# haoxiangsnr/Wave-U-Net-for-Speech-Enhancement

Measured on AMD Instinct MI355X. Metric: 16384-sample frames/sec fwd+bwd, 12-level Wave-U-Net, higher is better.
Workload: dtype f32 (levels >= 16 samples: 3 x f16 MFMA on hi/lo fp16 halves, fp32 accumulate; the rest f32 MFMA); 1 GPU; unet_basic 12-level, 16384-sample frames, batch=64 per GPU, fp32, training-mode forward + smooth_l1 + backward + fused HIP Adam step (BASELINE.json configs[2]; configs[3] when n_gpus>1); global_batch=64, frame=16384, parallelism=dp1

## Files before the change

### wave-u-net-for-speech-enhancement_amd/csrc/wunet_backward.cpp

```cpp
#include "wunet_host.h"
#include "wunet_elementwise.h"
#include "wunet_tiny.h"
#include "wunet_h3_elem.h"
#include "wunet_input_grad.h"

using namespace wunet_host;

namespace {
#ifndef WUNET_EMU
__global__ void stamp_kernel(unsigned long long* p) { *p = wall_clock64(); }
unsigned long long* g_stamps = nullptr;
bool stamps_on()
{
    static const bool on = getenv("WUNET_STAMP") != nullptr;
    if (on && !g_stamps && (hipMalloc(&g_stamps, 128 * sizeof(unsigned long long)) != hipSuccess || hipMemset(g_stamps, 0, 128 * sizeof(unsigned long long)) != hipSuccess)) g_stamps = nullptr;
    return on && g_stamps;
}
#define WUNET_STAMP(stream_, slot_) { if (stamps_on()) hipLaunchKernelGGL(stamp_kernel, dim3(1), dim3(1), 0, stream_, g_stamps + (slot_)); }
#else
#define WUNET_STAMP(stream_, slot_) {}
#endif

bool dx_stays_split(const wunet_ctx* c, int i)
{
    if (i < 1 || i > c->n) return false;
    const LayerPlan& l = c->ly[i];
    return l.d.ksplit > 1 && l.L >= 4 && c->ly[i - 1].L >= 4;
}

bool enc_gz_off()
{
    static const bool off = getenv("WUNET_NO_ENC_GZ") != nullptr;
    return off;
}
bool pa_swap_on()
{
    static const int on = getenv("WUNET_PA_SWAP") ? atoi(getenv("WUNET_PA_SWAP")) : 1;
    return on != 0;
}

bool bwd_tiny(const wunet_ctx* c, int i) { return c->ly[i].L < 4; }
bool bwd_one_block(const wunet_ctx* c, int i) { return c->ly[i].a_split == 1 && (size_t)c->B * c->ly[i].L <= 4 * WUNET_THREADS; }
bool bwd_fuse(const wunet_ctx* c, int i) { return !bwd_tiny(c, i) && i < c->NL - 1 && !(i > 0 && c->ly[i].h3d) && bwd_one_block(c, i); }

bool upt_handoff(const wunet_ctx* c, int q) { return q > c->n && q < c->NL && c->ly[q].upt; }
bool upt_handoff_sound(const wunet_ctx* c, int q)
{
    const LayerPlan& l = c->ly[q];
    return l.src0 == q - 1 && l.h3d && l.d.ksplit == 1 && c->ly[q - 1].h3d && !bwd_tiny(c, q - 1) && !bwd_fuse(c, q - 1);
}

enum { DG_NONE = 0, DG_H3 = 1, DG_SCALAR = 2, DG_FP32 = 3 };
struct BwdLayerPlan {
    bool tiny;
    bool fuse;
    bool gz_h3;
    bool gz_in_wgrad;
    bool e0;
    int pa_mode;
    const char* pa_name;
    double g_src_bytes;
    bool stores_g;
    bool swap;
    bool g1_split;
    bool fin_in_gz;
    int gz_mode;
    int dgrad;
    bool dx_split, dx_sum;
    bool upt;
    double pa_bytes() const { return 4.0 + g_src_bytes + (stores_g ? 4.0 : 0.0); }
    double gz_bytes() const { return 4.0 + (gz_mode == GZ_G ? 4.0 : g_src_bytes); }
};
BwdLayerPlan bwd_layer_plan(const wunet_ctx* c, int i)
{
    const LayerPlan& l = c->ly[i];
    const int NL = c->NL, n = c->n;
    BwdLayerPlan q{};
    q.tiny = bwd_tiny(c, i);
    q.fuse = bwd_fuse(c, i);
    q.gz_h3 = i > 0 && l.h3d;
    q.gz_in_wgrad = i == 0 && !q.tiny && !l.h3d && !l.h3w && l.w.wsplit && !bwd_one_block(c, i);
    q.e0 = c->e0 && q.gz_in_wgrad && !q.fuse && l.cin == 1 && l.taps == 15 && l.L >= 16 && !dx_stays_split(c, 1) && n >= 1;
    const bool recompute = q.gz_h3 && !q.fuse && !q.tiny;
    q.stores_g = true;
    if (i == NL - 1) {
        q.pa_mode = A_HEAD; q.pa_name = "pass_a_kernel<HEAD>"; q.g_src_bytes = 0.0; q.gz_mode = GZ_HEAD;
        q.stores_g = !recompute;
    } else if (i >= n && upt_handoff(c, i + 1)) {
        q.pa_mode = A_UPH; q.pa_name = "pass_a_kernel<UPH>"; q.g_src_bytes = 4.0; q.gz_mode = GZ_UPH;
        q.stores_g = false;
    } else if (i >= n) {
        q.pa_mode = A_UP; q.pa_name = "pass_a_kernel<UP>"; q.g_src_bytes = 8.0; q.gz_mode = GZ_G;
    } else {
        q.g1_split = dx_stays_split(c, i + 1);
        q.pa_mode = A_ENC; q.pa_name = q.e0 ? "pass_a_kernel<ENC, e0>" : "pass_a_kernel<ENC>"; q.g_src_bytes = 6.0; q.gz_mode = GZ_ENC;
        q.stores_g = !(!enc_gz_off() && recompute && !q.g1_split) && !q.e0;
    }
    if (q.stores_g) q.gz_mode = GZ_G;
    q.swap = pa_swap_on() && l.a_split > 1 && !q.tiny;
    q.fin_in_gz = !q.fuse && q.gz_h3 && l.a_split * l.cout <= WUNET_GZ_FIN_LOADS && l.cout <= WUNET_GZ_FIN_C;
    q.dgrad = i == 0 ? DG_NONE : l.h3d ? DG_H3 : q.tiny ? DG_SCALAR : DG_FP32;
    q.dx_split = q.dgrad != DG_NONE && q.dgrad != DG_SCALAR && l.d.ksplit > 1;
    q.dx_sum = q.dx_split && !dx_stays_split(c, i);
    q.upt = upt_handoff(c, i);
    return q;
}

int first_layer_gz_source(const wunet_ctx* c)
{
    const BwdLayerPlan q = bwd_layer_plan(c, 0);
    return q.e0 ? IG_ENC : q.gz_in_wgrad ? IG_G : IG_GZ;
}

struct BwdCall {
    wunet_ctx* c; float* ws; const float* const* params; float* const* grads; const float* noisy;
    hipStream_t st, sd;
    wunet_ctx::Side* side;
};

int head_backward(const BwdCall& k, void* workspace, const float* enhanced, const float* grad_enhanced)
{
    wunet_ctx* c = k.c; float* ws = k.ws; const hipStream_t st = k.st;
    if (k.side->packed_ws == workspace && k.sd != st) {
        k.side->packed_ws = nullptr;
        if (hipStreamWaitEvent(st, k.side->ev_pack, 0) != hipSuccess) return fail(WUNET_E_RUNTIME, "waiting for the weight packs failed");
    } else {
        k.side->packed_ws = nullptr;
        const int rc = launch_backward_packs(c, k.params, ws, st);
        if (rc) return rc;
    }
    const LayerPlan& l = c->ly[c->NL - 1];
    HeadBwdArgs h{};
    h.z = ws + l.z; h.a = ws + l.a; h.s = ws + l.s; h.in = k.noisy; h.out = enhanced; h.gout = grad_enhanced;
    h.gh = ws + c->gh_off; h.part = ws + c->hpart_off; h.B = c->B; h.C = c->ci; h.T = c->T; h.logT = ilog2(c->T);
    WUNET_LAUNCH(head_bwd_kernel, dim3(c->head_blocks), dim3(WUNET_THREADS), 0, st, h);
    WUNET_CHECK_LAUNCH();
    return WUNET_OK;
}

int pass_a(const BwdCall& k, int i, const BwdLayerPlan& q, int fz)
{
    wunet_ctx* c = k.c; float* ws = k.ws; const hipStream_t st = k.st;
    const int NL = c->NL, n = c->n;
    const LayerPlan& l = c->ly[i];
    PassAArgs p{};
    p.z = ws + l.z; p.a = ws + l.a; p.s = ws + l.s; p.mean = ws + l.mean; p.rstd = ws + l.rstd;
    p.gpre = q.stores_g ? ws + l.g : nullptr; p.part = ws + c->bpart_off; p.pmax = q.gz_h3 ? ws + c->bmax_off : nullptr;
    p.B = c->B; p.C = l.cout; p.L = l.L; p.logL = l.logL; p.Lt = l.Lt;
    p.swap = q.swap ? 1 : 0;
    const dim3 ga(p.swap ? l.a_split : l.cout, p.swap ? l.cout : l.a_split);
    if (q.fuse) {
        p.gamma = k.params[4 * i + 2]; p.dgamma = k.grads[4 * i + 2]; p.dbeta = k.grads[4 * i + 3]; p.dbias = k.grads[4 * i + 1];
        p.k1 = ws + l.k1; p.k2 = ws + l.k2; p.k3 = ws + l.k3; p.count = (double)c->B * l.Lt; p.frozen = fz;
    }
    prof_begin(st, q.pa_name, 0.0, (double)c->B * l.cout * l.L * q.pa_bytes() + (q.pa_mode == A_HEAD ? 4.0 * c->B * l.L : 0.0));
    if (q.pa_mode == A_HEAD) {
        p.g0 = ws + c->gh_off; p.g1 = k.params[4 * NL]; p.hpart = ws + c->hpart2_off;
        WUNET_LAUNCH(pass_a_kernel<A_HEAD>, ga, dim3(WUNET_THREADS), 0, st, p);
    } else if (q.pa_mode == A_UPH) {
        const LayerPlan& nx = c->ly[i + 1];
        p.g0 = ws + nx.dxh; p.sp = ws + nx.usp; p.ntiles = (int)(((size_t)c->B * nx.L + 255) / 256); p.tpr = l.L >> 7;
        WUNET_LAUNCH(pass_a_kernel<A_UPH>, ga, dim3(WUNET_THREADS), 0, st, p);
    } else if (q.pa_mode == A_UP) {
        const LayerPlan& nx = c->ly[i + 1];
        p.g0 = ws + nx.dx; p.Cg0 = nx.cin;
        p.up_scale = (float)(l.Lt - 1) / (float)(2 * l.Lt - 1);
        if (q.tiny) WUNET_LAUNCH(pass_a_scalar_kernel<A_UP>, ga, dim3(WUNET_THREADS), 0, st, p);
        else if (q.fuse) WUNET_LAUNCH((pass_a_kernel<A_UP, true>), ga, dim3(WUNET_THREADS), 0, st, p);
        else WUNET_LAUNCH(pass_a_kernel<A_UP>, ga, dim3(WUNET_THREADS), 0, st, p);
    } else {
        const LayerPlan& dc = c->ly[2 * n - i];
        const LayerPlan& nx = c->ly[i + 1];
        p.g0 = ws + dc.dx; p.Cg0 = dc.cin; p.coff = dc.c0; p.g1 = ws + nx.dx;
        if (q.g1_split) {
            p.g1 = ws + c->spart_off; p.g1_splits = nx.d.ksplit; p.g1_stride = (size_t)c->B * nx.cin * nx.L;
        }
        if (q.e0) { p.x0 = k.noisy; p.e0rows = ws + c->e0part_off; }
        if (q.tiny) WUNET_LAUNCH(pass_a_scalar_kernel<A_ENC>, ga, dim3(WUNET_THREADS), 0, st, p);
        else if (q.e0) WUNET_LAUNCH((pass_a_kernel<A_ENC, false, false, true>), ga, dim3(WUNET_THREADS), 0, st, p);
        else if (q.fuse && p.g1_splits > 1) WUNET_LAUNCH((pass_a_kernel<A_ENC, true, true>), ga, dim3(WUNET_THREADS), 0, st, p);
        else if (q.fuse) WUNET_LAUNCH((pass_a_kernel<A_ENC, true>), ga, dim3(WUNET_THREADS), 0, st, p);
        else if (p.g1_splits > 1) WUNET_LAUNCH((pass_a_kernel<A_ENC, false, true>), ga, dim3(WUNET_THREADS), 0, st, p);
        else WUNET_LAUNCH(pass_a_kernel<A_ENC>, ga, dim3(WUNET_THREADS), 0, st, p);
    }
    prof_end(st);
    WUNET_CHECK_LAUNCH();
    return WUNET_OK;
}

int finalize_and_gz(const BwdCall& k, int i, const BwdLayerPlan& q, int fz)
{
    wunet_ctx* c = k.c; float* ws = k.ws; const hipStream_t st = k.st;
    const LayerPlan& l = c->ly[i];
    BnBwdArgs b{};
    b.part = ws + c->bpart_off; b.rows = l.a_split; b.gamma = k.params[4 * i + 2]; b.mean = ws + l.mean; b.rstd = ws + l.rstd;
    b.dgamma = k.grads[4 * i + 2]; b.dbeta = k.grads[4 * i + 3]; b.dbias = k.grads[4 * i + 1]; b.k1 = ws + l.k1; b.k2 = ws + l.k2; b.k3 = ws + l.k3;
    b.C = l.cout; b.count = (double)c->B * l.Lt; b.frozen = fz;
    b.pmax = q.gz_h3 ? ws + c->bmax_off : nullptr; b.bound = ws + c->bound_off;
    if (q.e0) { b.e0rows = ws + c->e0part_off; b.dw0 = k.grads[0]; }
    if (!q.fin_in_gz) {
        WUNET_LAUNCH(bn_finalize_bwd_kernel, dim3(l.cout), dim3(WUNET_THREADS), 0, st, b);
        WUNET_CHECK_LAUNCH();
    }
    const size_t n4 = (size_t)c->B * l.cout * l.L / 4;
    if (q.gz_h3) {
        const int c8 = (l.cout + 7) / 8;
        const size_t nt = (size_t)c->B * c8 * (l.L / 4);
        size_t hb = (nt + WUNET_THREADS - 1) / WUNET_THREADS;
        if (hb > 8192) hb = 8192;
        prof_begin(st, "gz_split_h3_kernel", 0.0, (double)c->B * l.cout * l.L * (q.gz_bytes() + (c->bf ? 2.0 : 4.0)));
        GzHeadArgs hd{};
        if (q.gz_mode != GZ_G) { hd.a = ws + l.a; hd.s = ws + l.s; }
        if (q.gz_mode == GZ_HEAD) { hd.gh = ws + c->gh_off; hd.wh = k.params[4 * c->NL]; }
        if (q.gz_mode == GZ_UPH) hd.gq = ws + c->ly[i + 1].dxh;
        if (q.gz_mode == GZ_ENC) {
            const LayerPlan& dc = c->ly[2 * c->n - i];
            hd.gd = ws + dc.dx; hd.Cg0 = dc.cin; hd.coff = dc.c0; hd.ge = ws + c->ly[i + 1].dx;
        }
#define WUNET_GZ_LAUNCH(FIN_, GM_, BF_)                                                                                                               \
    WUNET_LAUNCH((gz_split_h3_kernel<FIN_, GM_, BF_>), dim3((unsigned)hb), dim3(WUNET_THREADS), 0, st, (const float*)(ws + l.g), (const float*)(ws + l.z), \
                 (const float*)(ws + l.k1), (const float*)(ws + l.k2), (const float*)(ws + l.k3), (const float*)(ws + c->bound_off),                 \
                 ws + c->h3_slot + 8 + 4 * i, reinterpret_cast<wunet_half*>(ws + l.gzh), reinterpret_cast<wunet_half*>(ws + l.gzl),                  \
                 c->B, l.cout, c8, l.L, l.logL, l.Lt, b, hd)
#define WUNET_GZ_MODE(GM_)                                                                                                                            \
    case GM_:                                                                                                                                         \
        if (q.fin_in_gz) { if (c->bf) WUNET_GZ_LAUNCH(true, GM_, true); else WUNET_GZ_LAUNCH(true, GM_, false); }                                     \
        else { if (c->bf) WUNET_GZ_LAUNCH(false, GM_, true); else WUNET_GZ_LAUNCH(false, GM_, false); }                                               \
        break;
        switch (q.gz_mode) { WUNET_GZ_MODE(GZ_G) WUNET_GZ_MODE(GZ_HEAD) WUNET_GZ_MODE(GZ_ENC) WUNET_GZ_MODE(GZ_UPH) }
#undef WUNET_GZ_MODE
#undef WUNET_GZ_LAUNCH
        prof_end(st);
    } else if (q.tiny) {
        WUNET_LAUNCH(gz_scalar_kernel, dim3((unsigned)((n4 * 4 + WUNET_THREADS - 1) / WUNET_THREADS) + 1), dim3(WUNET_THREADS), 0, st, (const float*)(ws + l.g),
                     (const float*)(ws + l.z), (const float*)(ws + l.k1), (const float*)(ws + l.k2), (const float*)(ws + l.k3), l.cout, l.logL,
                     (size_t)c->B * l.cout * l.L, ws + l.g);
    } else if (!q.gz_in_wgrad) {
        size_t blocks = (n4 + WUNET_THREADS - 1) / WUNET_THREADS;
        if (blocks > 8192) blocks = 8192;
        WUNET_LAUNCH(gz_materialize_kernel, dim3((unsigned)blocks), dim3(WUNET_THREADS), 0, st, (const float*)(ws + l.g), (const float*)(ws + l.z),
                     (const float*)(ws + l.k1), (const float*)(ws + l.k2), (const float*)(ws + l.k3), l.cout, l.logL, n4, ws + l.g, l.Lt);
    }
    WUNET_CHECK_LAUNCH();
    return WUNET_OK;
}

int sum_dx_splits(const BwdCall& k, const LayerPlan& l)
{
    const size_t nd = (size_t)k.c->B * l.cin * l.L;
    size_t blocks = (nd + WUNET_THREADS - 1) / WUNET_THREADS;
    if (blocks > 2048) blocks = 2048;
    WUNET_LAUNCH(split_sum_kernel, dim3((unsigned)blocks), dim3(WUNET_THREADS), 0, k.st, (const float*)(k.ws + k.c->spart_off), l.d.ksplit, nd, k.ws + l.dx, (const float*)nullptr, 1, 0);
    WUNET_CHECK_LAUNCH();
    return WUNET_OK;
}

int data_gradient(const BwdCall& k, int i, const BwdLayerPlan& q)
{
    wunet_ctx* c = k.c; float* ws = k.ws; const hipStream_t st = k.st;
    const LayerPlan& l = c->ly[i];
    float* const dx = q.dx_split ? ws + c->spart_off : ws + l.dx;
    if (q.dgrad == DG_H3) {
        ConvH3Upt up{};
        if (q.upt) {
            up.c0 = l.c0; up.up_scale = (float)(l.Lt / 2 - 1) / (float)(l.Lt - 1);
            up.uh_out = ws + l.dxh; up.uh_spill = ws + l.usp;
        }
        const int rc = launch_conv_h3(l.taps, l.h3d_mrep, l.h3d_mtp, l.h3d_sps, reinterpret_cast<wunet_half*>(ws + l.gzh), reinterpret_cast<wunet_half*>(ws + l.gzl),
                                      reinterpret_cast<const wunet_half*>(ws + c->h3_wb_hi) + l.h3d_wpk,
                                      reinterpret_cast<const wunet_half*>(ws + c->h3_wb_lo) + l.h3d_wpk, nullptr, ws + c->h3_slot + 8 + 4 * i,
                                      ws + c->fslot_off + (size_t)WUNET_SLOT_FLOATS * i + 2,
                                      dx, nullptr, c->B, l.cin, l.cout, l.h3d_nch, l.L, st, ws + l.gzp, nullptr, nullptr,
                                      nullptr, c->bf, l.h3d_ntt, nullptr, q.upt ? &up : nullptr);
        if (rc) return rc;
        WUNET_CHECK_LAUNCH();
    } else if (q.dgrad == DG_SCALAR) {
        const size_t nd = (size_t)c->B * l.cin * l.L;
        WUNET_LAUNCH(tiny_conv_kernel, dim3((unsigned)((nd + WUNET_THREADS - 1) / WUNET_THREADS)), dim3(WUNET_THREADS), 0, st,
                     (const float*)(ws + l.g), k.params[4 * i], ws + l.dx, c->B, l.cout, l.cin, l.L, l.logL, l.taps, 1);
        WUNET_CHECK_LAUNCH();
    } else if (q.dgrad == DG_FP32) {
        const ConvArgs a = make_conv_args(ws + l.g, l.cout, ws + c->wpkb_off + l.d_wpk, nullptr, dx, nullptr, c->B, l.cin, l.L, l.taps, l.d,
                                          (size_t)c->B * l.cin * l.L);
        const int rc = launch_conv(l.taps, a, l.d, st);
        if (rc) return rc;
        WUNET_CHECK_LAUNCH();
    }
    return q.dx_sum ? sum_dx_splits(k, l) : WUNET_OK;
}

int weight_gradient(const BwdCall& k, int i, const BwdLayerPlan& q)
{
    wunet_ctx* c = k.c; float* ws = k.ws; const hipStream_t sd = k.sd;
    const int NL = c->NL;
    const LayerPlan& l = c->ly[i];
    if (sd != k.st && hipStreamWaitEvent(sd, k.side->ev_fork, 0) != hipSuccess) return fail(WUNET_E_RUNTIME, "fork onto the weight-gradient stream failed");
    WUNET_STAMP(sd, 2 * i + 1)
    if (i == NL - 1) {
        WUNET_LAUNCH(rows_sum_kernel, dim3(2), dim3(WUNET_THREADS), 0, sd,
                     (const float*)(ws + c->hpart_off), c->head_blocks, 2, k.grads[4 * NL] + c->ci, 1, k.grads[4 * NL + 1]);
        WUNET_CHECK_LAUNCH();
        WUNET_LAUNCH(rows_sum_kernel, dim3(c->ci), dim3(WUNET_THREADS), 0, sd,
                     (const float*)(ws + c->hpart2_off), l.a_split, c->ci, k.grads[4 * NL], c->ci, k.grads[4 * NL + 1]);
        WUNET_CHECK_LAUNCH();
    }
    if (q.e0) return WUNET_OK;
    const float* xin = i == 0 ? k.noisy : ws + l.xin;
    const size_t nw = (size_t)l.cout * l.cin * l.taps;
    if (q.tiny) {
        WUNET_LAUNCH(tiny_wgrad_kernel, dim3((unsigned)((nw + WUNET_THREADS - 1) / WUNET_THREADS)), dim3(WUNET_THREADS), 0, sd,
                     (const float*)(ws + l.g), xin, k.grads[4 * i], c->B, l.cin, l.cout, l.L, l.taps);
        WUNET_CHECK_LAUNCH();
        return WUNET_OK;
    }
    int rc;
    if (l.h3w)
        rc = launch_wgrad_h3(l, reinterpret_cast<const wunet_half*>(ws + l.xh), reinterpret_cast<const wunet_half*>(ws + l.xl),
                             reinterpret_cast<const wunet_half*>(ws + l.gzh), reinterpret_cast<const wunet_half*>(ws + l.gzl),
                             ws + c->h3_slot + 8 + 4 * i, ws + c->fslot_off + (size_t)WUNET_SLOT_FLOATS * i,
                             ws + c->wgpart_off, c->B, sd, c->bf);
    else {
        WgradArgs w = make_wgrad_args(xin, ws + l.g, ws + c->wgpart_off, c->B, l.cin, l.cout, l.L, l.taps, l.w.cps);
        if (q.gz_in_wgrad) {
            w.z = ws + l.z; w.k1 = ws + l.k1; w.k2 = ws + l.k2; w.k3 = ws + l.k3; w.Lt = l.Lt;
        }
        rc = launch_wgrad_any(l.taps, w, l.w, sd);
    }
    if (rc) return rc;
    WUNET_CHECK_LAUNCH();
    if (l.h3w) {
        WgradH3ReduceArgs ra{};
        ra.part = ws + c->wgpart_off; ra.part_stride = h3w_part_stride(l); ra.splits = l.h3w_ksplit; ra.dw = k.grads[4 * i];
// ... 150 lines not shown
```

### wave-u-net-for-speech-enhancement_amd/csrc/wunet_elementwise.h

```cpp
#pragma once
#include "wunet_dev.h"

struct PackDesc {
    const float* w;
    float* dst;
    int Cout, Cin, taps;
    int M;
    int CP;
    int mtiles;
    int transposed;
};

#define WUNET_MAX_CONV_LAYERS 34
struct PackTable { PackDesc d[WUNET_MAX_CONV_LAYERS]; };

static __global__ __launch_bounds__(WUNET_THREADS) void pack_weights_kernel(PackTable tab)
{
    const PackDesc& d = tab.d[blockIdx.y];
    const int total = d.mtiles * d.CP * d.taps * 16;
    const int kc = d.transposed ? d.Cout : d.Cin;
    for (int idx = blockIdx.x * WUNET_THREADS + threadIdx.x; idx < total; idx += gridDim.x * WUNET_THREADS) {
        const int i = idx & 15;
        int r = idx >> 4;
        const int t = r % d.taps; r /= d.taps;
// ... 356 lines not shown
    size_t p = beg + threadIdx.x;
    for (; p + 3 * WUNET_THREADS < end; p += 4 * WUNET_THREADS) {
        float o[4], go[4], xi[4];
#pragma unroll
        for (int u = 0; u < 4; ++u) { o[u] = A.out[p + u * WUNET_THREADS]; go[u] = A.gout[p + u * WUNET_THREADS]; xi[u] = A.in[p + u * WUNET_THREADS]; }
#pragma unroll
        for (int u = 0; u < 4; ++u) {
            const float g = go[u] * (1.0f - o[u] * o[u]);
            A.gh[p + u * WUNET_THREADS] = g;
            sb += (double)g;
            sin_ += (double)g * (double)xi[u];
        }
    }
    for (; p < end; p += WUNET_THREADS) {
        const float o = A.out[p];
        const float g = A.gout[p] * (1.0f - o * o);
        A.gh[p] = g;
        sb += (double)g;
        sin_ += (double)g * (double)A.in[p];
    }
    block_sum2(sb, sin_, red);
    if (threadIdx.x == 0) {
        A.part[(size_t)blockIdx.x * 2] = (float)sin_;
        A.part[(size_t)blockIdx.x * 2 + 1] = (float)sb;
    }
}

static __global__ __launch_bounds__(WUNET_THREADS) void rows_sum_kernel(const float* part, int rows, int n, float* out0, int n0, float* out1)
{
    __shared__ double red[2 * WUNET_THREADS];
    const int j = blockIdx.x;
    double s = 0.0, dummy = 0.0;
    for (int r = threadIdx.x; r < rows; r += WUNET_THREADS) s += (double)part[(size_t)r * n + j];
    block_sum2(s, dummy, red);
    if (threadIdx.x == 0) {
        if (j < n0) out0[j] = (float)s; else out1[j - n0] = (float)s;
    }
}

enum { A_HEAD = 0, A_UP = 1, A_ENC = 2, A_UPH = 3 };

__device__ __forceinline__ void wunet_uph_edges(const float* sp, int C, int ntiles, int tpr, int b, int c, int l, int L, float* gq_at_l, float& g_first, float& g_last)
{
    const int tile = b * tpr + (l >> 7);
    if ((l & 127) == 0 && l > 0) { g_first += sp[(size_t)c * ntiles + tile - 1]; gq_at_l[0] = g_first; }
    if ((l & 127) == 124 && l + 4 < L) { g_last += sp[((size_t)C + c) * ntiles + tile + 1]; gq_at_l[3] = g_last; }
}

struct WunetUpT { float c0[10], c1[10]; bool fast; };
__device__ __forceinline__ void wunet_upT_coords(int l, int Lt, float up_scale, WunetUpT& U)
{
    const int j0 = 2 * l - 4;
    U.fast = l >= 4 && l + 8 <= Lt;
    if (U.fast) {
#pragma unroll
        for (int k = 3; k <= 12; ++k) {
            int i0, i1;
            wunet_up_coord(j0 + k, Lt, up_scale, i0, i1, U.c0[k - 3], U.c1[k - 3]);
            U.fast = U.fast && i0 == ((j0 + k - 1) >> 1) && i1 == i0 + 1;
        }
    }
}
__device__ __forceinline__ void wunet_upT_row(const float* row, int l, int Lo, int Lot, int Lt, float up_scale, const WunetUpT& U, float (&g)[4])
{
    const int j0 = 2 * l - 4;
    g[0] = g[1] = g[2] = g[3] = 0.0f;
    if (U.fast) {
        const float dm = row[j0 + 3];
        const wunet_f4 da = wunet_ld4(row + j0 + 4), db = wunet_ld4(row + j0 + 8);
        const float dl = row[j0 + 12];
        const float d[10] = {dm, da[0], da[1], da[2], da[3], db[0], db[1], db[2], db[3], dl};
#pragma unroll
        for (int m = 0; m < 4; ++m) {
            g[m] += U.c1[2 * m] * d[2 * m];
            g[m] += U.c1[2 * m + 1] * d[2 * m + 1];
            g[m] += U.c0[2 * m + 2] * d[2 * m + 2];
            g[m] += U.c0[2 * m + 3] * d[2 * m + 3];
        }
        return;
    }
#pragma unroll
    for (int k = 2; k <= 12; ++k) {
        const int j = j0 + k;
        if (j >= 0 && j < Lot) {
            const float dv = row[j];
            int i0, i1; float l0, l1;
            wunet_up_coord(j, Lt, up_scale, i0, i1, l0, l1);
#pragma unroll
            for (int m = 0; m < 4; ++m) {
                const float w = (i0 == l + m ? l0 : 0.0f) + (i1 == l + m ? l1 : 0.0f);
                g[m] += w * dv;
            }
        }
    }
    (void)Lo;
}

struct PassAArgs {
    const float* z;
    const float* a;
    const float* s;
    const float* mean;
    const float* rstd;
    float* gpre;
    float* part;
    float* pmax;
    float* hpart;
    const float* g0;
    const float* g1;
    int Cg0;
    int g1_splits;
    size_t g1_stride;
    int coff;
    int B, C, L, logL;
    float up_scale;
    int swap;
    int Lt;
    const float* sp;
    int ntiles, tpr;
    const float* x0; float* e0rows;
    const float* gamma; float* dgamma; float* dbeta; float* dbias; float* k1; float* k2; float* k3; double count;
    int frozen;
};

__device__ __forceinline__ void block_reduce_pass_a(double& s1, double& s2, double& s3, bool want3, float& mg, float& mz, double* red)
{
    const int tid = threadIdx.x;
#pragma unroll
    for (int m = 32; m > 0; m >>= 1) {
        s1 += wunet_shfl_xor_d(s1, m);
        s2 += wunet_shfl_xor_d(s2, m);
        if (want3) s3 += wunet_shfl_xor_d(s3, m);
        mg = fmaxf(mg, wunet_shfl_xor(mg, m));
        mz = fmaxf(mz, wunet_shfl_xor(mz, m));
    }
    if ((tid & 63) == 0) {
        const int w = tid >> 6;
        red[w] = s1; red[WUNET_WAVES + w] = s2; red[2 * WUNET_WAVES + w] = s3;
        red[3 * WUNET_WAVES + w] = (double)mg; red[4 * WUNET_WAVES + w] = (double)mz;
    }
    __syncthreads();
    s1 = (red[0] + red[1]) + (red[2] + red[3]);
    s2 = (red[WUNET_WAVES] + red[WUNET_WAVES + 1]) + (red[WUNET_WAVES + 2] + red[WUNET_WAVES + 3]);
    s3 = (red[2 * WUNET_WAVES] + red[2 * WUNET_WAVES + 1]) + (red[2 * WUNET_WAVES + 2] + red[2 * WUNET_WAVES + 3]);
    mg = fmaxf(fmaxf((float)red[3 * WUNET_WAVES], (float)red[3 * WUNET_WAVES + 1]), fmaxf((float)red[3 * WUNET_WAVES + 2], (float)red[3 * WUNET_WAVES + 3]));
    mz = fmaxf(fmaxf((float)red[4 * WUNET_WAVES], (float)red[4 * WUNET_WAVES + 1]), fmaxf((float)red[4 * WUNET_WAVES + 2], (float)red[4 * WUNET_WAVES + 3]));
}

template <int MODE, bool E0 = false>
struct PassALoads {
    wunet_f4 z, g;
    float e0, e1;
    float d[MODE == A_UP ? 13 : 1];
    wunet_f4 xw[E0 ? 5 : 1];
    size_t zi; int b, l;
};

template <int MODE, bool FUSE = false, bool G1S = false, bool E0 = false>
__global__ __launch_bounds__(WUNET_THREADS) void pass_a_kernel(PassAArgs A)
{
    static_assert(!E0 || (MODE == A_ENC && !FUSE && !G1S), "E0: the first layer's gradient assembly");
    __shared__ double red[5 * WUNET_WAVES];
    __shared__ float e0x[E0 ? WUNET_WAVES * 48 : 1];
    float w1[E0 ? 15 : 1], w2[E0 ? 15 : 1], w3[E0 ? 15 : 1];
    if (E0) {
#pragma unroll
        for (int k = 0; k < 15; ++k) w1[E0 ? k : 0] = w2[E0 ? k : 0] = w3[E0 ? k : 0] = 0.0f;
    }
    const int c = A.swap ? blockIdx.y : blockIdx.x;
    const unsigned by = A.swap ? blockIdx.x : blockIdx.y, ny = A.swap ? gridDim.x : gridDim.y;
    const size_t total4 = ((size_t)A.B * A.L) >> 2;
    const size_t per = (total4 + ny - 1) / ny;
    const size_t beg = (size_t)by * per, end = beg + per < total4 ? beg + per : total4;
    const float a = A.a[c], s = A.s[c], mu = A.mean[c], rstd = A.rstd[c];
    const float wh = MODE == A_HEAD ? A.g1[c] : 0.0f;
    const float gam = FUSE ? A.gamma[c] : 0.0f;
    double s1 = 0.0, s2 = 0.0, s3 = 0.0;
    float mg = 0.0f, mz = 0.0f;
    wunet_f4 keep_g = wunet_f4{0.f, 0.f, 0.f, 0.f}, keep_z = keep_g;
    size_t keep_i = 0;
    int keep_l = 0;
    bool have = false;

    auto load = [&](size_t q4, PassALoads<MODE, E0>& t) {
        const size_t p = q4 << 2;
        t.b = (int)(p >> A.logL); t.l = (int)(p & (size_t)(A.L - 1));
        const int b = t.b, l = t.l;
        t.zi = ((size_t)b * A.C + c) * A.L + l;
        t.z = wunet_ld4(A.z + t.zi);
        t.e0 = t.e1 = 0.0f;
        if (MODE == A_HEAD) t.g = wunet_ld4(A.g0 + (size_t)b * A.L + l);
        else if (MODE == A_UPH) {
            t.g = wunet_ld4(A.g0 + t.zi);
            const int tile = b * A.tpr + (l >> 7);
            t.e0 = A.sp[(size_t)c * A.ntiles + (tile > 0 ? tile - 1 : 0)];
            t.e1 = A.sp[((size_t)A.C + c) * A.ntiles + (tile + 1 < A.ntiles ? tile + 1 : tile)];
        }
        else if (MODE == A_ENC) {
            t.g = wunet_ld4(A.g0 + ((size_t)b * A.Cg0 + A.coff + c) * A.L + l);
            const float* ge = A.g1 + ((size_t)b * A.C + c) * (A.L >> 1) + (l >> 1);
            float e0, e1;
            if (G1S) {
                e0 = e1 = 0.0f;
                int k = 0;
                for (; k + 4 <= A.g1_splits; k += 4) {
                    const float2 t0 = *reinterpret_cast<const float2*>(ge + (size_t)k * A.g1_stride);
                    const float2 t1 = *reinterpret_cast<const float2*>(ge + (size_t)(k + 1) * A.g1_stride);
                    const float2 t2 = *reinterpret_cast<const float2*>(ge + (size_t)(k + 2) * A.g1_stride);
                    const float2 t3 = *reinterpret_cast<const float2*>(ge + (size_t)(k + 3) * A.g1_stride);
                    e0 += t0.x; e0 += t1.x; e0 += t2.x; e0 += t3.x;
                    e1 += t0.y; e1 += t1.y; e1 += t2.y; e1 += t3.y;
                }
                if (k < A.g1_splits) {
                    const int last = A.g1_splits - 1;
                    const float2 t0 = *reinterpret_cast<const float2*>(ge + (size_t)k * A.g1_stride);
                    const float2 t1 = *reinterpret_cast<const float2*>(ge + (size_t)(k + 1 < last ? k + 1 : last) * A.g1_stride);
                    const float2 t2 = *reinterpret_cast<const float2*>(ge + (size_t)(k + 2 < last ? k + 2 : last) * A.g1_stride);
                    e0 += t0.x; e1 += t0.y;
                    e0 += k + 1 <= last ? t1.x : 0.0f; e1 += k + 1 <= last ? t1.y : 0.0f;
                    e0 += k + 2 <= last ? t2.x : 0.0f; e1 += k + 2 <= last ? t2.y : 0.0f;
                }
            } else { const float2 tt = *reinterpret_cast<const float2*>(ge); e0 = tt.x; e1 = tt.y; }
            t.e0 = e0; t.e1 = e1;
            if (E0) {
                const float* xr = A.x0 + (size_t)b * A.L;
#pragma unroll
                for (int v = 0; v < 5; ++v) {
                    const int lv = l - 8 + 4 * v;
                    const bool ok = lv >= 0 && lv < A.L;
                    t.xw[E0 ? v : 0] = wunet_sel4(ok, wunet_ld4(xr + (ok ? lv : 0)));
                }
            }
        } else {
            const int Lo = 2 * A.L;
            const float* row = A.g0 + ((size_t)b * A.Cg0 + c) * Lo;
            const int j0 = 2 * l - 4;
#pragma unroll
            for (int v = 0; v < 3; ++v) {
                const int jv = j0 + 4 * v;
                const bool ok = jv >= 0 && jv < Lo;
                const wunet_f4 tt = wunet_sel4(ok, wunet_ld4(row + (ok ? jv : 0)));
                t.d[(MODE == A_UP ? 4 * v : 0)] = tt[0]; t.d[(MODE == A_UP ? 4 * v + 1 : 0)] = tt[1];
                t.d[(MODE == A_UP ? 4 * v + 2 : 0)] = tt[2]; t.d[(MODE == A_UP ? 4 * v + 3 : 0)] = tt[3];
            }
            t.d[MODE == A_UP ? 12 : 0] = (j0 + 12 < Lo) ? row[j0 + 12] : 0.0f;
            t.g = wunet_f4{0.f, 0.f, 0.f, 0.f};
        }
    };

    auto compute = [&](const PassALoads<MODE, E0>& t) {
        const int b = t.b, l = t.l;
        const wunet_f4 z = t.z;
        float g[4];
        if (MODE == A_HEAD) {
#pragma unroll
            for (int j = 0; j < 4; ++j) {
                g[j] = wh * t.g[j];
                s3 += (double)(t.g[j] * wunet_lrelu(a * z[j] + s));
            }
        } else if (MODE == A_UPH) {
            float* const gq = const_cast<float*>(A.g0) + t.zi;
            g[0] = t.g[0]; g[1] = t.g[1]; g[2] = t.g[2]; g[3] = t.g[3];
            const bool first = (l & 127) == 0 && l > 0, last = (l & 127) == 124 && l + 4 < A.L;
            g[0] += first ? t.e0 : 0.0f;
            g[3] += last ? t.e1 : 0.0f;
            if (first) gq[0] = g[0];
            if (last) gq[3] = g[3];
        } else if (MODE == A_ENC) {
            g[0] = t.g[0] + t.e0; g[1] = t.g[1]; g[2] = t.g[2] + t.e1; g[3] = t.g[3];
        } else {
            const int Lot = 2 * A.Lt;
            const float* d = t.d;
            const float dlast = t.d[MODE == A_UP ? 12 : 0];
            const int j0 = 2 * l - 4;
            g[0] = g[1] = g[2] = g[3] = 0.0f;
            bool fast = l >= 4 && l + 8 <= A.Lt;
            float c0[10], c1[10];
            if (fast) {
#pragma unroll
                for (int k = 3; k <= 12; ++k) {
                    int i0, i1;
                    wunet_up_coord(j0 + k, A.Lt, A.up_scale, i0, i1, c0[k - 3], c1[k - 3]);
                    fast = fast && i0 == ((j0 + k - 1) >> 1) && i1 == i0 + 1;
                }
            }
            if (fast) {
#pragma unroll
                for (int m = 0; m < 4; ++m) {
                    g[m] += c1[2 * m] * d[MODE == A_UP ? 2 * m + 3 : 0];
                    g[m] += c1[2 * m + 1] * d[MODE == A_UP ? 2 * m + 4 : 0];
                    g[m] += c0[2 * m + 2] * d[MODE == A_UP ? 2 * m + 5 : 0];
                    g[m] += c0[2 * m + 3] * (m == 3 ? dlast : d[MODE == A_UP ? (m == 3 ? 0 : 2 * m + 6) : 0]);
                }
            } else
#pragma unroll
            for (int k = 2; k <= 12; ++k) {
                const int j = j0 + k;
                const float dv = k < 12 ? d[MODE == A_UP ? (k < 12 ? k : 0) : 0] : dlast;
                if (j >= 0 && j < Lot) {
                    int i0, i1; float l0, l1;
                    wunet_up_coord(j, A.Lt, A.up_scale, i0, i1, l0, l1);
#pragma unroll
                    for (int m = 0; m < 4; ++m) {
                        const float w = (i0 == l + m ? l0 : 0.0f) + (i1 == l + m ? l1 : 0.0f);
                        g[m] += w * dv;
                    }
                }
            }
        }
        wunet_f4 go;
#pragma unroll
        for (int j = 0; j < 4; ++j) {
            float gv = g[j];
            if (!(a * z[j] + s > 0.0f)) gv *= WUNET_SLOPE;
            const bool pad = l + j >= A.Lt;
            if (pad) gv = 0.0f;
            const float zc = pad ? 0.0f : z[j] - mu;
            go[j] = gv;
            s1 += (double)gv;
            s2 += (double)(gv * (zc * rstd));
            mg = fmaxf(mg, fabsf(gv));
            mz = fmaxf(mz, fabsf(zc));
        }
        if (E0) {
            float xs[20];
#pragma unroll
            for (int v = 0; v < 5; ++v) { xs[4 * v] = t.xw[E0 ? v : 0][0]; xs[4 * v + 1] = t.xw[E0 ? v : 0][1]; xs[4 * v + 2] = t.xw[E0 ? v : 0][2]; xs[4 * v + 3] = t.xw[E0 ? v : 0][3]; }
#pragma unroll
            for (int j = 0; j < 4; ++j) {
                const bool pad = l + j >= A.Lt;
                const float zz = pad ? 0.0f : z[j], one = pad ? 0.0f : 1.0f;
#pragma unroll
                for (int k = 0; k < 15; ++k) {
                    w1[E0 ? k : 0] = fmaf(go[j], xs[j + k + 1], w1[E0 ? k : 0]);
                    w2[E0 ? k : 0] = fmaf(zz, xs[j + k + 1], w2[E0 ? k : 0]);
                }
                if (c == 0) {
#pragma unroll
                    for (int k = 0; k < 15; ++k) w3[E0 ? k : 0] = fmaf(one, xs[j + k + 1], w3[E0 ? k : 0]);
                }
            }
        }
        if (FUSE) { keep_g = go; keep_z = z; keep_i = t.zi; keep_l = l; have = true; }
        else if (A.gpre) wunet_st4(A.gpre + t.zi, go);
    };

    for (size_t q4 = beg + threadIdx.x; q4 < end; q4 += 2 * WUNET_THREADS) {
        PassALoads<MODE, E0> t0, t1;
        const bool two = !FUSE && q4 + WUNET_THREADS < end;
        load(q4, t0);
        if (!FUSE) load(two ? q4 + WUNET_THREADS : q4, t1);
        compute(t0);
        if (two) compute(t1);
    }
    const bool want_max = A.pmax != nullptr;
    if (E0) {
#pragma unroll
        for (int q = 0; q < 45; ++q) {
            float v = q < 15 ? w1[E0 ? q : 0] : q < 30 ? w2[E0 ? q - 15 : 0] : w3[E0 ? q - 30 : 0];
            v = wunet_row16_sum(v);
            v += wunet_shfl_xor(v, 16);
            v += wunet_shfl_xor(v, 32);
            if ((threadIdx.x & 63) == 0) e0x[E0 ? (threadIdx.x >> 6) * 48 + q : 0] = v;
        }
        __syncthreads();
        if (threadIdx.x < 45) {
            const int q = threadIdx.x;
            A.e0rows[((size_t)by * A.C + c) * 48 + q] = (e0x[E0 ? q : 0] + e0x[E0 ? 48 + q : 0]) + (e0x[E0 ? 96 + q : 0] + e0x[E0 ? 144 + q : 0]);
        }
    }
    block_reduce_pass_a(s1, s2, s3, MODE == A_HEAD, mg, mz, red);
    if (FUSE) {
        const double t1 = (double)(float)s1, t2 = (double)(float)s2;
        const double m1 = A.frozen ? 0.0 : t1 / A.count, m2 = A.frozen ? 0.0 : t2 / A.count;
        const double ar = (double)gam * (double)rstd;
        const float k1 = (float)ar, k2 = (float)(-ar * m2 * (double)rstd), k3 = (float)(ar * m2 * (double)rstd * (double)mu - ar * m1);
        if (threadIdx.x == 0) {
            A.dgamma[c] = (float)t2;
            A.dbeta[c] = (float)t1;
            A.dbias[c] = A.frozen ? (float)(ar * t1) : 0.0f;
            A.k1[c] = k1; A.k2[c] = k2; A.k3[c] = k3;
        }
        if (have) {
            wunet_f4 o;
#pragma unroll
            for (int j = 0; j < 4; ++j) o[j] = keep_l + j < A.Lt ? k1 * keep_g[j] + k2 * keep_z[j] + k3 : 0.0f;
            wunet_st4(A.gpre + keep_i, o);
        }
        return;
    }
    if (threadIdx.x == 0) {
        float* pr = A.part + ((size_t)by * A.C + c) * 2;
        pr[0] = (float)s1;
        pr[1] = (float)s2;
        if (want_max) {
            float* pm = A.pmax + ((size_t)by * A.C + c) * 2;
            pm[0] = mg;
            pm[1] = mz;
        }
        if (MODE == A_HEAD && A.hpart) A.hpart[(size_t)by * A.C + c] = (float)s3;
    }
}

struct BnBwdArgs {
    const float* part; int rows;
    const float* gamma; const float* mean; const float* rstd;
    float* dgamma; float* dbeta;
    float* dbias;
    float* k1; float* k2; float* k3;
    int C; double count;
    const float* pmax;
    float* bound;
    const float* e0rows;
    float* dw0;
    int frozen;
};

static __global__ __launch_bounds__(WUNET_THREADS) void bn_finalize_bwd_kernel(BnBwdArgs A)
{
    __shared__ double red[5 * WUNET_WAVES];
    const int c = blockIdx.x, tid = threadIdx.x;
    const float gam = A.gamma[c], rs = A.rstd[c], mu = A.mean[c];
    double s1 = 0.0, s2 = 0.0, s3 = 0.0;
    float mg = 0.0f, mz = 0.0f;
    for (int r = tid; r < A.rows; r += WUNET_THREADS) {
        const float2 pr = *reinterpret_cast<const float2*>(A.part + ((size_t)r * A.C + c) * 2);
        float2 pm = float2{0.0f, 0.0f};
        if (A.pmax) pm = *reinterpret_cast<const float2*>(A.pmax + ((size_t)r * A.C + c) * 2);
        s1 += (double)pr.x;
        s2 += (double)pr.y;
        mg = fmaxf(mg, pm.x);
        mz = fmaxf(mz, pm.y);
    }
    block_reduce_pass_a(s1, s2, s3, false, mg, mz, red);
    if (tid == 0) {
        const double m1 = A.frozen ? 0.0 : s1 / A.count, m2 = A.frozen ? 0.0 : s2 / A.count;
        const double a = (double)gam * (double)rs;
        A.dgamma[c] = (float)s2;
        A.dbeta[c] = (float)s1;
        A.dbias[c] = A.frozen ? (float)(a * s1) : 0.0f;
        A.k1[c] = (float)a;
        A.k2[c] = (float)(-a * m2 * (double)rs);
        A.k3[c] = (float)(a * m2 * (double)rs * (double)mu - a * m1);
        if (A.pmax) A.bound[c] = (float)(fabs(a) * (double)mg + fabs(a * m2 * (double)rs) * (double)mz + fabs(a * m1));
    }
    if (A.e0rows) {
        __shared__ double e0s[48];
        if (tid < 45) {
            double t = 0.0;
            for (int r0 = 0; r0 < A.rows; r0 += 32) {
                float v[32];
#pragma unroll
                for (int r = 0; r < 32; ++r) v[r] = A.e0rows[((size_t)(r0 + r < A.rows ? r0 + r : 0) * A.C + (tid < 30 ? c : 0)) * 48 + tid];
#pragma unroll
                for (int r = 0; r < 32; ++r) if (r0 + r < A.rows) t += (double)v[r];
            }
            e0s[tid] = t;
        }
        __syncthreads();
        if (tid < 15) {
            const double m1 = A.frozen ? 0.0 : s1 / A.count, m2 = A.frozen ? 0.0 : s2 / A.count;
            const double a = (double)gam * (double)rs;
            const float k1 = (float)a, k2 = (float)(-a * m2 * (double)rs), k3 = (float)(a * m2 * (double)rs * (double)mu - a * m1);
            A.dw0[c * 15 + tid] = (float)((double)k1 * e0s[tid] + (double)k2 * e0s[15 + tid] + (double)k3 * e0s[30 + tid]);
        }
    }
}

static __global__ __launch_bounds__(WUNET_THREADS) void wgrad_reduce_kernel(const float* part, int splits, size_t n, float* dw)
{
    __shared__ double red[16][16][4];
    const int og = threadIdx.x & 15, sl = threadIdx.x >> 4;
    const size_t n4 = n >> 2;
    for (size_t base = (size_t)blockIdx.x * 16; base < n4; base += (size_t)gridDim.x * 16) {
        const size_t i = base + og;
        double t0 = 0.0, t1 = 0.0, t2 = 0.0, t3 = 0.0;
        if (i < n4) {
            int r = sl;
            for (; r + 7 * 16 < splits; r += 8 * 16) {
                float a0 = 0.f, a1 = 0.f, a2 = 0.f, a3 = 0.f;
#pragma unroll
                for (int k = 0; k < 8; ++k) {
                    const wunet_f4 v = wunet_ld4(part + (size_t)(r + k * 16) * n + 4 * i);
                    a0 += v[0]; a1 += v[1]; a2 += v[2]; a3 += v[3];
                }
                t0 += (double)a0; t1 += (double)a1; t2 += (double)a2; t3 += (double)a3;
            }
            for (; r < splits; r += 16) {
                const wunet_f4 v = wunet_ld4(part + (size_t)r * n + 4 * i);
                t0 += (double)v[0]; t1 += (double)v[1]; t2 += (double)v[2]; t3 += (double)v[3];
            }
        }
        __syncthreads();
        red[sl][og][0] = t0; red[sl][og][1] = t1; red[sl][og][2] = t2; red[sl][og][3] = t3;
        __syncthreads();
        if (sl == 0 && i < n4) {
            double u0 = 0.0, u1 = 0.0, u2 = 0.0, u3 = 0.0;
#pragma unroll
            for (int k = 0; k < 16; ++k) { u0 += red[k][og][0]; u1 += red[k][og][1]; u2 += red[k][og][2]; u3 += red[k][og][3]; }
            wunet_f4 o;
            o[0] = (float)u0; o[1] = (float)u1; o[2] = (float)u2; o[3] = (float)u3;
            wunet_st4(dw + 4 * i, o);
        }
    }
    for (size_t i = (n4 << 2) + (size_t)blockIdx.x * WUNET_THREADS + threadIdx.x; i < n; i += (size_t)gridDim.x * WUNET_THREADS) {
        double tot = 0.0;
        for (int r = 0; r < splits; ++r) tot += (double)part[(size_t)r * n + i];
        dw[i] = (float)tot;
    }
}

template <int K>
__global__ __launch_bounds__(WUNET_THREADS) void conv_first_kernel(const float* x, const float* w, const float* bias, float* out,
                                                                    float* stats, int B, int Cout, int L, int logL,
                                                                    const float* ev_a, const float* ev_s, float* xrows, int Lt)
{
    constexpr int PAD = K / 2, NX = ((8 + 4 + PAD + 3) / 4) * 4;
    static_assert(PAD <= 8 && NX >= 8 + 4 + PAD, "window");
    const int lane = threadIdx.x & 63, wave = threadIdx.x >> 6;
    const size_t p = ((size_t)blockIdx.x * WUNET_THREADS + threadIdx.x) * 4;
    const int b = (int)(p >> logL), l0 = (int)(p & (size_t)(L - 1));
    const bool live = b < B;
// ... 379 lines not shown
```

Before: 12690 frames/s.

## Stage first-layer input windows in LDS and split ones-sum into extra block

The first-layer (e0) pass-A kernel now stages chunks of the noisy input into shared memory and reads each thread's 20-sample window from LDS, instead of doing five overlapping global vector loads per element. The ones-weighted accumulator (w3), which only channel 0 used to compute, moves to a dedicated extra grid column (c == C), so no channel carries the imbalance. Block reductions now sum 16-lane rows through shared memory rather than using cross-lane shuffles. The cost is more shared memory per block and extra barriers per chunk, which may reduce occupancy.

```diff
diff --git a/wave-u-net-for-speech-enhancement_amd/csrc/wunet_backward.cpp b/wave-u-net-for-speech-enhancement_amd/csrc/wunet_backward.cpp
--- a/wave-u-net-for-speech-enhancement_amd/csrc/wunet_backward.cpp
+++ b/wave-u-net-for-speech-enhancement_amd/csrc/wunet_backward.cpp
@@ -93,7 +93,8 @@
         q.pa_mode = A_UP; q.pa_name = "pass_a_kernel<UP>"; q.g_src_bytes = 8.0; q.gz_mode = GZ_G;
     } else {
         q.g1_split = dx_stays_split(c, i + 1);
-        q.pa_mode = A_ENC; q.pa_name = q.e0 ? "pass_a_kernel<ENC, e0>" : "pass_a_kernel<ENC>"; q.g_src_bytes = 6.0; q.gz_mode = GZ_ENC;
+        q.pa_mode = A_ENC; q.g_src_bytes = 6.0; q.gz_mode = GZ_ENC;
+        q.pa_name = q.e0 ? "pass_a_kernel<ENC, e0>" : q.g1_split && !q.fuse && !q.tiny ? "pass_a_kernel<ENC, g1s>" : "pass_a_kernel<ENC>";
         q.stores_g = !(!enc_gz_off() && recompute && !q.g1_split) && !q.e0;
     }
     if (q.stores_g) q.gz_mode = GZ_G;
@@ -177,7 +178,10 @@
         }
         if (q.e0) { p.x0 = k.noisy; p.e0rows = ws + c->e0part_off; }
         if (q.tiny) WUNET_LAUNCH(pass_a_scalar_kernel<A_ENC>, ga, dim3(WUNET_THREADS), 0, st, p);
-        else if (q.e0) WUNET_LAUNCH((pass_a_kernel<A_ENC, false, false, true>), ga, dim3(WUNET_THREADS), 0, st, p);
+        else if (q.e0) {
+            const dim3 ge(p.swap ? l.a_split : l.cout + 1, p.swap ? l.cout + 1 : l.a_split);
+            WUNET_LAUNCH((pass_a_kernel<A_ENC, false, false, true>), ge, dim3(WUNET_THREADS), 0, st, p);
+        }
         else if (q.fuse && p.g1_splits > 1) WUNET_LAUNCH((pass_a_kernel<A_ENC, true, true>), ga, dim3(WUNET_THREADS), 0, st, p);
         else if (q.fuse) WUNET_LAUNCH((pass_a_kernel<A_ENC, true>), ga, dim3(WUNET_THREADS), 0, st, p);
         else if (p.g1_splits > 1) WUNET_LAUNCH((pass_a_kernel<A_ENC, false, true>), ga, dim3(WUNET_THREADS), 0, st, p);
diff --git a/wave-u-net-for-speech-enhancement_amd/csrc/wunet_elementwise.h b/wave-u-net-for-speech-enhancement_amd/csrc/wunet_elementwise.h
--- a/wave-u-net-for-speech-enhancement_amd/csrc/wunet_elementwise.h
+++ b/wave-u-net-for-speech-enhancement_amd/csrc/wunet_elementwise.h
@@ -532,26 +532,105 @@
     wunet_f4 z, g;
     float e0, e1;
     float d[MODE == A_UP ? 13 : 1];
-    wunet_f4 xw[E0 ? 5 : 1];
     size_t zi; int b, l;
+    int xo;
 };
+
+#ifndef WUNET_E0_CHUNK4
+#ifdef WUNET_EMU
+#define WUNET_E0_CHUNK4 512
+#else
+#define WUNET_E0_CHUNK4 2048
+#endif
+#endif
+__device__ __forceinline__ void wunet_e0_stage(const float* x0, size_t n, size_t cb, size_t ce, float* xs)
+{
+    const int n4 = (int)(ce - cb) + 4;
+    for (int i0 = threadIdx.x; i0 < n4; i0 += 3 * WUNET_THREADS) {
+        wunet_f4 v[3];
+#pragma unroll
+        for (int u = 0; u < 3; ++u) {
+            const size_t p = 4 * cb + 4 * (size_t)(i0 + u * WUNET_THREADS);
+            const bool ok = i0 + u * WUNET_THREADS < n4 && p >= 8 && p - 8 < n;
+            v[u] = wunet_sel4(ok, wunet_ld4(x0 + (ok ? p - 8 : 0)));
+        }
+#pragma unroll
+        for (int u = 0; u < 3; ++u)
+            if (i0 + u * WUNET_THREADS < n4) wunet_st4(xs + 4 * (i0 + u * WUNET_THREADS), v[u]);
+    }
+}
+__device__ __forceinline__ void wunet_e0_window(const float* xs, int xo, int l, int L, float (&x)[20])
+{
+#pragma unroll
+    for (int v = 0; v < 5; ++v) {
+        const int lv = l - 8 + 4 * v;
+        const wunet_f4 t = wunet_sel4(lv >= 0 && lv < L, wunet_ld4(xs + xo + 4 * v));
+        x[4 * v] = t[0]; x[4 * v + 1] = t[1]; x[4 * v + 2] = t[2]; x[4 * v + 3] = t[3];
+    }
+}
+template <int N>
+__device__ __forceinline__ void wunet_e0_block_sums(const float (&w)[N], float* rows, float* out)
+{
+    static_assert(N <= 32, "one 32-float line per 16-lane row");
+#pragma unroll
+    for (int q = 0; q < N; ++q) {
+        const float v = wunet_row16_sum(w[q]);
+        if ((threadIdx.x & 15) == 0) rows[(threadIdx.x >> 4) * 32 + q] = v;
+    }
+    __syncthreads();
+    if (threadIdx.x < N) {
+        float ws[WUNET_WAVES];
+#pragma unroll
+        for (int k = 0; k < WUNET_WAVES; ++k) {
+            const float* r = rows + k * 128 + threadIdx.x;
+            ws[k] = (r[0] + r[32]) + (r[64] + r[96]);
+        }
+        out[threadIdx.x] = (ws[0] + ws[1]) + (ws[2] + ws[3]);
+    }
+}
 
 template <int MODE, bool FUSE = false, bool G1S = false, bool E0 = false>
 __global__ __launch_bounds__(WUNET_THREADS) void pass_a_kernel(PassAArgs A)
 {
     static_assert(!E0 || (MODE == A_ENC && !FUSE && !G1S), "E0: the first layer's gradient assembly");
     __shared__ double red[5 * WUNET_WAVES];
-    __shared__ float e0x[E0 ? WUNET_WAVES * 48 : 1];
-    float w1[E0 ? 15 : 1], w2[E0 ? 15 : 1], w3[E0 ? 15 : 1];
+    __shared__ float e0xs[E0 ? 4 * WUNET_E0_CHUNK4 + 16 : 4];
+    __shared__ float e0x[E0 ? 16 * 32 : 1];
+    float w1[E0 ? 15 : 1], w2[E0 ? 15 : 1];
     if (E0) {
 #pragma unroll
-        for (int k = 0; k < 15; ++k) w1[E0 ? k : 0] = w2[E0 ? k : 0] = w3[E0 ? k : 0] = 0.0f;
+        for (int k = 0; k < 15; ++k) w1[E0 ? k : 0] = w2[E0 ? k : 0] = 0.0f;
     }
     const int c = A.swap ? blockIdx.y : blockIdx.x;
     const unsigned by = A.swap ? blockIdx.x : blockIdx.y, ny = A.swap ? gridDim.x : gridDim.y;
     const size_t total4 = ((size_t)A.B * A.L) >> 2;
     const size_t per = (total4 + ny - 1) / ny;
     const size_t beg = (size_t)by * per, end = beg + per < total4 ? beg + per : total4;
+    size_t cb = beg;
+    if (E0 && c == A.C) {
+        float w3[15];
+#pragma unroll
+        for (int k = 0; k < 15; ++k) w3[k] = 0.0f;
+        for (; cb < end; cb += WUNET_E0_CHUNK4) {
+            const size_t ce = cb + WUNET_E0_CHUNK4 < end ? cb + WUNET_E0_CHUNK4 : end;
+            if (cb != beg) __syncthreads();
+            wunet_e0_stage(A.x0, (size_t)A.B * A.L, cb, ce, e0xs);
+            __syncthreads();
+            for (size_t q4 = cb + threadIdx.x; q4 < ce; q4 += WUNET_THREADS) {
+                const int l = (int)((q4 << 2) & (size_t)(A.L - 1));
+                float xs[20];
+                wunet_e0_window(e0xs, (int)(q4 - cb) << 2, l, A.L, xs);
+#pragma unroll
+                for (int j = 0; j < 4; ++j) {
+                    const float one = l + j >= A.Lt ? 0.0f : 1.0f;
+#pragma unroll
+                    for (int k = 0; k < 15; ++k) w3[k] = fmaf(one, xs[j + k + 1], w3[k]);
+                }
+            }
+        }
+        wunet_e0_block_sums<15>(w3, e0x, A.e0rows + (size_t)by * A.C * 48 + 30);
+        return;
+    }
     const float a = A.a[c], s = A.s[c], mu = A.mean[c], rstd = A.rstd[c];
     const float wh = MODE == A_HEAD ? A.g1[c] : 0.0f;
     const float gam = FUSE ? A.gamma[c] : 0.0f;
@@ -602,15 +681,7 @@
                 }
             } else { const float2 tt = *reinterpret_cast<const float2*>(ge); e0 = tt.x; e1 = tt.y; }
             t.e0 = e0; t.e1 = e1;
-            if (E0) {
-                const float* xr = A.x0 + (size_t)b * A.L;
-#pragma unroll
-                for (int v = 0; v < 5; ++v) {
-                    const int lv = l - 8 + 4 * v;
-                    const bool ok = lv >= 0 && lv < A.L;
-                    t.xw[E0 ? v : 0] = wunet_sel4(ok, wunet_ld4(xr + (ok ? lv : 0)));
-                }
-            }
+            if (E0) t.xo = (int)(q4 - cb) << 2;
         } else {
             const int Lo = 2 * A.L;
             const float* row = A.g0 + ((size_t)b * A.Cg0 + c) * Lo;
@@ -704,50 +775,47 @@
         }
         if (E0) {
             float xs[20];
-#pragma unroll
-            for (int v = 0; v < 5; ++v) { xs[4 * v] = t.xw[E0 ? v : 0][0]; xs[4 * v + 1] = t.xw[E0 ? v : 0][1]; xs[4 * v + 2] = t.xw[E0 ? v : 0][2]; xs[4 * v + 3] = t.xw[E0 ? v : 0][3]; }
+            wunet_e0_window(e0xs, t.xo, l, A.L, xs);
 #pragma unroll
             for (int j = 0; j < 4; ++j) {
-                const bool pad = l + j >= A.Lt;
-                const float zz = pad ? 0.0f : z[j], one = pad ? 0.0f : 1.0f;
+                const float zz = l + j >= A.Lt ? 0.0f : z[j];
 #pragma unroll
                 for (int k = 0; k < 15; ++k) {
                     w1[E0 ? k : 0] = fmaf(go[j], xs[j + k + 1], w1[E0 ? k : 0]);
                     w2[E0 ? k : 0] = fmaf(zz, xs[j + k + 1], w2[E0 ? k : 0]);
                 }
-                if (c == 0) {
-#pragma unroll
-                    for (int k = 0; k < 15; ++k) w3[E0 ? k : 0] = fmaf(one, xs[j + k + 1], w3[E0 ? k : 0]);
-                }
             }
         }
         if (FUSE) { keep_g = go; keep_z = z; keep_i = t.zi; keep_l = l; have = true; }
         else if (A.gpre) wunet_st4(A.gpre + t.zi, go);
     };
 
-    for (size_t q4 = beg + threadIdx.x; q4 < end; q4 += 2 * WUNET_THREADS) {
-        PassALoads<MODE, E0> t0, t1;
-        const bool two = !FUSE && q4 + WUNET_THREADS < end;
-        load(q4, t0);
-        if (!FUSE) load(two ? q4 + WUNET_THREADS : q4, t1);
-        compute(t0);
-        if (two) compute(t1);
-    }
+    auto trips = [&](size_t ce) {
+        for (size_t q4 = cb + threadIdx.x; q4 < ce; q4 += 2 * WUNET_THREADS) {
+            PassALoads<MODE, E0> t0, t1;
+            const bool two = !FUSE && q4 + WUNET_THREADS < end;
+            load(q4, t0);
+            if (!FUSE) load(two ? q4 + WUNET_THREADS : q4, t1);
+            compute(t0);
+            if (two) compute(t1);
+        }
+    };
+    if (E0) {
+        static_assert(WUNET_E0_CHUNK4 % (2 * WUNET_THREADS) == 0, "a chunk: whole double trips");
+        for (; cb < end; cb += WUNET_E0_CHUNK4) {
+            const size_t ce = cb + WUNET_E0_CHUNK4 < end ? cb + WUNET_E0_CHUNK4 : end;
+            if (cb != beg) __syncthreads();
+            wunet_e0_stage(A.x0, (size_t)A.B * A.L, cb, ce, e0xs);
+            __syncthreads();
+            trips(ce);
+        }
+    } else trips(end);
     const bool want_max = A.pmax != nullptr;
     if (E0) {
-#pragma unroll
-        for (int q = 0; q < 45; ++q) {
-            float v = q < 15 ? w1[E0 ? q : 0] : q < 30 ? w2[E0 ? q - 15 : 0] : w3[E0 ? q - 30 : 0];
-            v = wunet_row16_sum(v);
-            v += wunet_shfl_xor(v, 16);
-            v += wunet_shfl_xor(v, 32);
-            if ((threadIdx.x & 63) == 0) e0x[E0 ? (threadIdx.x >> 6) * 48 + q : 0] = v;
-        }
-        __syncthreads();
-        if (threadIdx.x < 45) {
-            const int q = threadIdx.x;
-            A.e0rows[((size_t)by * A.C + c) * 48 + q] = (e0x[E0 ? q : 0] + e0x[E0 ? 48 + q : 0]) + (e0x[E0 ? 96 + q : 0] + e0x[E0 ? 144 + q : 0]);
-        }
+        float w12[30];
+#pragma unroll
+        for (int q = 0; q < 30; ++q) w12[q] = q < 15 ? w1[E0 ? q : 0] : w2[E0 ? q - 15 : 0];
+        wunet_e0_block_sums<30>(w12, e0x, A.e0rows + ((size_t)by * A.C + c) * 48);
     }
     block_reduce_pass_a(s1, s2, s3, MODE == A_HEAD, mg, mz, red);
     if (FUSE) {
```

After: 12720 frames/s, median of 6. About the same (+0.2%).
